# mom-ocean/MOM6

Measured on AMD Instinct MI355X. Metric: simulated-days/wall-sec, higher is better.
Workload: dtype f64

## Files before the change

### include/mom6x.h

```cpp
#ifndef MOM6X_H
#define MOM6X_H

#include <stddef.h>
#include <stdint.h>

#ifdef __cplusplus
extern "C" {
#endif

#define MOM6X_ABI_VERSION 6

typedef struct mom6x_dims {
  int ni, nj, nk;
  int halo;
  int ioff, joff;
  int pitch;
  int slab;
  int i_glob0, j_glob0;
  int ni_glob, nj_glob;
  int reentrant_x, reentrant_y;
} mom6x_dims;

int mom6x_dims_init(mom6x_dims *d, int ni, int nj, int nk, int halo);

// ... 206 lines not shown
int mom6x_prof_reset(mom6x_ctx *ctx);
int mom6x_prof_filter(mom6x_ctx *ctx, const char *prefix);
int mom6x_prof_report(mom6x_ctx *ctx, char *buf, int buflen);

int mom6x_dev_alloc(mom6x_ctx *ctx, double **p, size_t n_doubles);
int mom6x_dev_free(mom6x_ctx *ctx, double *p);
int mom6x_dev_copy(mom6x_ctx *ctx, double *dst, const double *src, size_t n_doubles);
int mom6x_upload(mom6x_ctx *ctx, double *dev, const double *host_f, int stagger, int nk);
int mom6x_download(mom6x_ctx *ctx, double *host_f, const double *dev, int stagger, int nk);


int mom6x_continuity_init(mom6x_ctx *ctx, const mom6x_continuity_params *p);

int mom6x_continuity_stats(mom6x_ctx *ctx, int mode, unsigned long long *out3);

int mom6x_continuity_PPM(mom6x_ctx *ctx,
    const double *u, const double *v, const double *hin, double *h,
    double *uh, double *vh, double dt,
    const double *uhbt, const double *vhbt,
    const double *visc_rem_u, const double *visc_rem_v,
    double *u_cor, double *v_cor, const mom6x_BT_cont *BT_cont,
    double *du_cor, double *dv_cor);


int mom6x_barotropic_init(mom6x_ctx *ctx, const mom6x_barotropic_params *p);

int mom6x_btcalc(mom6x_ctx *ctx, const double *h, const double *h_u, const double *h_v);
int mom6x_btcalc_strict(mom6x_ctx *ctx, const double *h, const double *h_u, const double *h_v);

int mom6x_bt_mass_source(mom6x_ctx *ctx, const double *h, const double *eta, int set_cor);

int mom6x_set_dtbt(mom6x_ctx *ctx, const double *pbce, double gtot_est, double SSH_add,
                   double *dtbt_out);

int mom6x_set_dtbt_pbce_eta(mom6x_ctx *ctx, const double *pbce, const double *eta, double SSH_add, double *dtbt_out);
int mom6x_set_dtbt_pbce(mom6x_ctx *ctx, const double *pbce, double *dtbt_out);

int mom6x_btstep(mom6x_ctx *ctx,
    const double *U_in, const double *V_in, const double *eta_in, double dt,
    const double *bc_accel_u, const double *bc_accel_v,
    const double *taux, const double *tauy, const double *pbce,
    const double *eta_PF_in, const double *U_Cor, const double *V_Cor,
    double *accel_layer_u, double *accel_layer_v, double *eta_out,
    double *uhbtav, double *vhbtav,
    const double *visc_rem_u, const double *visc_rem_v,
    const mom6x_BT_cont *BT_cont,
    const double *taux_bot, const double *tauy_bot,
    const double *uh0, const double *vh0, const double *u_uh0, const double *v_vh0,
    double *etaav);

int mom6x_btstep_warnings(mom6x_ctx *ctx, int reset, long long *count, double *info);

double *mom6x_barotropic_field(mom6x_ctx *ctx, int which);
int mom6x_barotropic_dtbt(mom6x_ctx *ctx, double *get, const double *set);

int mom6x_CoriolisAdv_init(mom6x_ctx *ctx, const mom6x_coriolis_params *p);
int mom6x_CorAdCalc(mom6x_ctx *ctx, const double *u, const double *v, const double *h,
                    const double *uh, const double *vh, double *CAu, double *CAv);

int mom6x_PressureForce_init(mom6x_ctx *ctx, const mom6x_pgf_params *p, const double *Rlay,
                             const double *g_prime);
int mom6x_PressureForce(mom6x_ctx *ctx, const double *h, double *PFu, double *PFv,
                        double *pbce, double *eta);
int mom6x_ALE_PLM_edge_values(mom6x_ctx *ctx, const double *h, const double *Q, int bdry_extrap, double *Q_t, double *Q_b);
int mom6x_ALE_PPM_edge_values(mom6x_ctx *ctx, const double *h, const double *Q, int bdry_extrap, double *Q_t, double *Q_b);
int mom6x_PressureForce_set_tv(mom6x_ctx *ctx, const double *T, const double *S, const mom6x_eos_params *eos);

int mom6x_hor_visc_init(mom6x_ctx *ctx, const mom6x_hor_visc_params *p);
int mom6x_horizontal_viscosity(mom6x_ctx *ctx, const double *u, const double *v, const double *h,
                               double *diffu, double *diffv);

enum mom6x_remap_scheme { MOM6X_REMAP_PCM = 0, MOM6X_REMAP_PLM = 2, MOM6X_REMAP_PPM_H4 = 4, MOM6X_REMAP_PPM_IH4 = 5 };
typedef struct mom6x_remapping_params {
  int    scheme;
  int    boundary_extrapolation;
  int    force_bounds_in_subcell;
  int    force_bounds_in_target;
  int    om4_remap_via_sub_cells;
  int    answer_date;
  double h_neglect;
  double h_neglect_edge;
} mom6x_remapping_params;

int mom6x_ALE_remap_tracers(mom6x_ctx *ctx, const mom6x_remapping_params *p, const double *h_old, const double *h_new,
                            double *const *fields, int nfields);
int mom6x_ALE_remap_set_h_vel(mom6x_ctx *ctx, const double *h_new, double *h_u, double *h_v);
int mom6x_ALE_remap_velocities(mom6x_ctx *ctx, const mom6x_remapping_params *p, const double *h_old_u, const double *h_old_v,
                               const double *h_new_u, const double *h_new_v, double *u, double *v);
int mom6x_ALE_remap_velocities_from_h(mom6x_ctx *ctx, const mom6x_remapping_params *p, const double *h_old, const double *h_new,
                                      double *u, double *v);
int mom6x_ALE_remap_velocities_conserve_ke(mom6x_ctx *ctx, const mom6x_remapping_params *p, const double *h_old_u,
                                           const double *h_old_v, const double *h_new_u, const double *h_new_v,
                                           double *u, double *v);
typedef struct mom6x_regrid_zstar_params {
  double min_thickness;
  double old_grid_weight;
  double depth_of_time_filter_shallow;
  double depth_of_time_filter_deep;
  double Z_ref;
} mom6x_regrid_zstar_params;
int mom6x_ALE_regrid_zstar(mom6x_ctx *ctx, const mom6x_regrid_zstar_params *p, const double *coordinateResolution,
                           const double *h, double *h_new, double *dzRegrid);

enum mom6x_interp_scheme {
  MOM6X_INTERP_P1M_H2 = 0,
  MOM6X_INTERP_PLM = 3, MOM6X_INTERP_PPM_H4 = 5
// ... 247 lines not shown
```

### mom6_amd/abi.py

```python
import ctypes as C
import os

_HERE = os.path.dirname(os.path.abspath(__file__))
LIB_PATH = os.path.join(_HERE, "lib", "libmom6x.so")

c_double_p = C.POINTER(C.c_double)


class Dims(C.Structure):
    _fields_ = [
        ("ni", C.c_int), ("nj", C.c_int), ("nk", C.c_int), ("halo", C.c_int),
        ("ioff", C.c_int), ("joff", C.c_int), ("pitch", C.c_int), ("slab", C.c_int),
        ("i_glob0", C.c_int), ("j_glob0", C.c_int), ("ni_glob", C.c_int), ("nj_glob", C.c_int),
        ("reentrant_x", C.c_int), ("reentrant_y", C.c_int),
    ]

    @property
    def nrows(self):
        return self.nj + 2 * self.halo + 1

    def shape2(self):
        return (self.nrows, self.pitch)

    def shape3(self, nk=None):
# ... 362 lines not shown


class RK2Params(C.Structure):
    _fields_ = [("be", C.c_double), ("begw", C.c_double), ("split_bottom_stress", C.c_int),
                ("BT_use_layer_fluxes", C.c_int), ("store_CAu", C.c_int), ("visc_rem_dt_bug", C.c_int), ("remap_aux", C.c_int),
                ("no_BT_cont", C.c_int)]


def rk2_params_default():
    p = RK2Params()
    p.be, p.begw = 0.6, 0.0
    p.split_bottom_stress = 0
    p.BT_use_layer_fluxes = p.store_CAu = p.visc_rem_dt_bug = 1
    p.remap_aux = 0
    p.no_BT_cont = 0
    return p


VERTVISC_COEF_HOOK = C.CFUNCTYPE(C.c_int, C.c_void_p, C.c_int, C.c_void_p, C.c_void_p, C.c_void_p, C.c_double)
HOR_VISC_HOOK = C.CFUNCTYPE(C.c_int, C.c_void_p, C.c_void_p, C.c_void_p, C.c_void_p, C.c_void_p, C.c_void_p,
                            C.c_void_p, C.c_void_p)


class RK2Hooks(C.Structure):
    _fields_ = [("user", C.c_void_p), ("vertvisc_coef", VERTVISC_COEF_HOOK), ("horizontal_viscosity", HOR_VISC_HOOK)]


RK2_FIELDS = ["CAu", "CAv", "CAu_pred", "CAv_pred", "PFu", "PFv", "diffu", "diffv", "visc_rem_u", "visc_rem_v",
              "u_accel_bt", "v_accel_bt", "u_av", "v_av", "h_av", "pbce", "eta", "eta_PF", "uhbt", "vhbt",
              "taux_bot", "tauy_bot", "BT_h_u", "BT_h_v"]
RK2_HAVE_ETA, RK2_HAVE_DIFFU, RK2_HAVE_U2, RK2_HAVE_CAU, RK2_HAVE_UH, RK2_HAVE_H2 = 1, 2, 4, 8, 16, 32
RK2_FIELDS_2D = {"eta", "eta_PF", "uhbt", "vhbt", "taux_bot", "tauy_bot"}


METRICS = [
    "mask2dT", "mask2dCu", "mask2dCv", "mask2dBu",
    "dxT", "dyT", "IdxT", "IdyT",
    "dxCu", "dyCu", "IdxCu", "IdyCu",
    "dxCv", "dyCv", "IdxCv", "IdyCv",
    "dxBu", "dyBu", "IdxBu", "IdyBu",
    "areaT", "IareaT", "areaBu", "IareaBu",
    "areaCu", "areaCv", "IareaCu", "IareaCv",
    "dy_Cu", "dx_Cv", "bathyT", "CoriolisBu", "Coriolis2Bu",
]
G = {n: i for i, n in enumerate(METRICS)}
G_COUNT = len(METRICS)

MOM6X_OK = 0

_lib = None


ABI_VERSION = 6


def load_library(path=None):
    global _lib
    if _lib is not None and path is None:
        return _lib
    p = path or LIB_PATH
    if not os.path.exists(p):
        raise RuntimeError(
            f"mom6_amd: HIP extension {p} is missing; run `python -c 'import __graft_entry__ as g; g.build()'`. "
            "There is no CPU fallback for the product path.")
    lib = C.CDLL(p, mode=C.RTLD_GLOBAL)
    if lib.mom6x_abi_version() != ABI_VERSION:
        raise RuntimeError(f"mom6_amd: {p} has ABI version {lib.mom6x_abi_version()}, this host mirror was written for "
                           f"{ABI_VERSION} (include/mom6x.h MOM6X_ABI_VERSION); rebuild the library")
    lib.mom6x_last_error.restype = C.c_char_p
    lib.mom6x_ctx_stream.restype = C.c_void_p
    lib.mom6x_ctx_dims.restype = C.POINTER(Dims)
    lib.mom6x_ctx_metrics_dev.restype = C.c_void_p
    for name in ("mom6x_barotropic_field", "mom6x_rk2_field"):
        if hasattr(lib, name):
            getattr(lib, name).restype = C.c_void_p
    if path is None:
        _lib = lib
    return lib


class Mom6xError(RuntimeError):
    pass


def check(lib, rc):
    if rc != MOM6X_OK:
        msg = lib.mom6x_last_error()
        raise Mom6xError(f"mom6x error {rc}: {msg.decode() if msg else ''}")
```

### mom6_amd/csrc/barotropic.hip

```cpp
#include <algorithm>
#include <type_traits>
#include <vector>
#include <cmath>
#include "mom6x_dev.h"

void halo_wrap(mom6x_ctx *c, double *const *fields, const int *staggers, const int *nks, int n);

enum BTW {
  W_q = 0, W_DCor_u, W_DCor_v, W_gtot_E, W_gtot_W, W_gtot_N, W_gtot_S, W_eta, W_eta_PF,
  W_Cor_ref_u, W_Cor_ref_v, W_BT_force_u, W_BT_force_v, W_ubt, W_vbt, W_bt_rem_u, W_bt_rem_v,
  W_uhbt0, W_vhbt0, W_ubt_Cor, W_vbt_Cor, W_uhbt, W_vhbt, W_u_accel_bt, W_v_accel_bt,
  W_eta_src, W_e_anom, W_eta_sum, W_eta_wtd, W_ubt_wtd, W_vbt_wtd, W_eta_pred,
  W_uh0sum, W_vh0sum, W_ubt0, W_vbt0,
  W_f4u, W_f4u_2, W_f4u_3, W_f4u_4, W_f4v, W_f4v_2, W_f4v_3, W_f4v_4,
  W_BTCu,
  W_BTCv = W_BTCu + 10,
  W_BTtmp = W_BTCv + 10,
  W_uhn = W_BTtmp + 12,
  W_vhn,
  W_ubt2, W_vbt2, W_eta_pred2,
  W_COUNT
};

enum BTC { B_FA_EE = 0, B_FA_E0, B_FA_W0, B_FA_WW, B_uBT_WW, B_uBT_EE, B_crvW, B_crvE, B_uh_WW, B_uh_EE };

struct BTState {
  double *frhatu, *frhatv, *IDatu, *IDatv, *ubtav, *vbtav, *eta_cor, *q_D, *D_u_Cor, *D_v_Cor;
  double *work;
  int nstep_last;
  unsigned long long *warn;
  double *warn_info;
  bool la_defer, la_pending;
  const double *la_pbce;
  double la_underflow;
  bool fr_defer, fr_pending;
  const double *fr_hu, *fr_hv;
};

namespace {

__device__ __forceinline__ double *wp(double *work, const Dm &d, int m) { return work + (size_t)m * d.slab; }

__device__ __forceinline__ double find_uhbt(double u, const double *__restrict__ B, size_t c, size_t slab) {
  if (u == 0.0) return 0.0;
  const double uEE = B[B_uBT_EE * slab + c];
  if (u < uEE) return (u - uEE) * B[B_FA_EE * slab + c] + B[B_uh_EE * slab + c];
  if (u < 0.0) return u * (B[B_FA_E0 * slab + c] + B[B_crvE * slab + c] * (u * u));
  const double uWW = B[B_uBT_WW * slab + c];
  if (u <= uWW) return u * (B[B_FA_W0 * slab + c] + B[B_crvW * slab + c] * (u * u));
  return (u - uWW) * B[B_FA_WW * slab + c] + B[B_uh_WW * slab + c];
}

__global__ void k_bt_init_static(Dm d, const double *__restrict__ G, double Z_to_H, double Mean_SL,
                                 double cor_scale, double H_subroundoff, double *q_D, double *D_u_Cor,
                                 double *D_v_Cor, double *IDatu, double *IDatv) {
  const int i = -1 + blockIdx.x * blockDim.x + threadIdx.x;
  const int j = -1 + blockIdx.y * blockDim.y + threadIdx.y;
  if (i > d.ni - 1 || j > d.nj - 1) return;
  const int st = d.pitch;
  const size_t c = ix2(d, i, j);
  const double *bathyT = gm(G, d, MOM6X_G_bathyT), *areaT = gm(G, d, MOM6X_G_areaT), *mT = gm(G, d, MOM6X_G_mask2dT);
  const double *mCu = gm(G, d, MOM6X_G_mask2dCu), *mCv = gm(G, d, MOM6X_G_mask2dCv), *fBu = gm(G, d, MOM6X_G_CoriolisBu);
  if (j >= 0) {
    D_u_Cor[c] = 0.5 * (dmax(Mean_SL + bathyT[c + 1], 0.0) + dmax(Mean_SL + bathyT[c], 0.0)) * Z_to_H;
    if (mCu[c] > 0.) IDatu[c] = mCu[c] * 2.0 / (Z_to_H * ((bathyT[c + 1] + bathyT[c]) + 2.0 * Mean_SL));
    else IDatu[c] = 0.;
  }
  if (i >= 0) {
    D_v_Cor[c] = 0.5 * (dmax(Mean_SL + bathyT[c + st], 0.0) + dmax(Mean_SL + bathyT[c], 0.0)) * Z_to_H;
    if (mCv[c] > 0.) IDatv[c] = mCv[c] * 2.0 / (Z_to_H * ((bathyT[c + st] + bathyT[c]) + 2.0 * Mean_SL));
    else IDatv[c] = 0.;
  }
  if (mT[c] + mT[c + st] + mT[c + 1] + mT[c + 1 + st] > 0.) {
    q_D[c] = 0.25 * (cor_scale * fBu[c]) * ((areaT[c] + areaT[c + 1 + st]) + (areaT[c + 1] + areaT[c + st])) /
// ... 160 lines not shown
  const size_t c = ix2(d, i, j), slab = (size_t)d.slab;
  const double subroundoff = 1e-30;
  const double mC = gm(G, d, DIR ? MOM6X_G_mask2dCv : MOM6X_G_mask2dCu)[c];
  double Ihattot = 0.0;
  if (HF) {
    double hattot = 0.0;
    for (int k = 0; k < nz; k++) hattot = hattot + A.hf[c + (size_t)k * slab];
    Ihattot = mC / (hattot + A.h_neglect);
  }
#define FRH(k) (HF ? A.hf[c + (size_t)(k) * slab] * Ihattot : A.frhat[c + (size_t)(k) * slab])
  double Iwt_tot = 1.0;
  if (!A.wt_uv_bug) {
    double tot = 0.0;
    for (int k = 0; k < nz; k++) {
      double vr = dmin(A.visc_rem[c + k * slab], 1.);
      vr = dmax(vr, 1. - 0.5 * A.Instep / (vr + subroundoff));
      vr = dmax(vr, 0.);
      const double w = FRH(k) * vr;
      tot = (k == 0) ? w : (tot + w);
    }
    Iwt_tot = tot;
    if (fabs(tot) > 0.0) Iwt_tot = mC / tot;
  }
  double ubt_Cor = 0.0, gm_ = 0.0, gp_ = 0.0, uh0sum = 0.0, ubt0 = 0.0, ubt = 0.0, av_rem = 0.0;
  double BT_force = 0.0;
  if (mC > 0.0) {
    BT_force = A.tau[c] * A.RZ_to_H * A.IDat[c] * A.visc_rem[c];
    if (A.tau_bot) BT_force = BT_force - A.tau_bot[c] * A.RZ_to_H * A.IDat[c];
  }
  for (int k = 0; k < nz; k++) {
    const size_t f = c + k * slab;
    const double vrem = A.visc_rem[f], frh = FRH(k);
    double vr = dmin(vrem, 1.);
    vr = dmax(vr, 1. - 0.5 * A.Instep / (vr + subroundoff));
    vr = dmax(vr, 0.);
    double wt = frh * vr;
    if (!A.wt_uv_bug) wt = wt * Iwt_tot;
    ubt_Cor = ubt_Cor + wt * A.U_Cor[f];
    gm_ = gm_ + A.pbce[f] * wt;
    gp_ = gp_ + A.pbce[f + st] * wt;
    if (A.uh0) {
      uh0sum = uh0sum + A.uh0[f];
      ubt0 = ubt0 + (A.visc_rem_u_uh0 ? wt : frh) * A.u_uh0[f];
    }
    ubt = ubt + wt * A.U_in[f];
    BT_force = BT_force + wt * A.bc_accel[f];
    av_rem = av_rem + frh * vrem;
  }
#undef FRH
  A.ubt_Cor[c] = ubt_Cor;
  A.gtot_m[c] = gm_;
  A.gtot_p[c + st] = gp_;
  if (A.uh0) { A.uh0sum[c] = uh0sum; A.ubt0[c] = ubt0; }
  if (fabs(ubt) < A.vel_underflow) ubt = 0.0;
  A.ubt[c] = ubt;
  A.BT_force[c] = BT_force;
  double bt_rem;
  if (A.strong_drag) {
    bt_rem = mC * ((A.nstep * av_rem) / (1.0 + (A.nstep - 1) * av_rem));
  } else {
    bt_rem = 0.0;
    if (mC * av_rem > 0.0) bt_rem = mC * pow(av_rem, A.Instep);
  }
  A.bt_rem[c] = bt_rem;
}

__global__ void k_btcont_copy(Dm d, mom6x_BT_cont BT, double *tmp) {
  const int i = -1 + blockIdx.x * blockDim.x + threadIdx.x;
  const int j = -1 + blockIdx.y * blockDim.y + threadIdx.y;
  if (i > d.ni - 1 || j > d.nj - 1) return;
  const size_t c = ix2(d, i, j), slab = (size_t)d.slab;
  if (j >= 0) {
    tmp[0 * slab + c] = BT.uBT_EE[c]; tmp[1 * slab + c] = BT.uBT_WW[c]; tmp[2 * slab + c] = BT.FA_u_EE[c];
    tmp[3 * slab + c] = BT.FA_u_E0[c]; tmp[4 * slab + c] = BT.FA_u_W0[c]; tmp[5 * slab + c] = BT.FA_u_WW[c];
  }
  if (i >= 0) {
    tmp[6 * slab + c] = BT.vBT_NN[c]; tmp[7 * slab + c] = BT.vBT_SS[c]; tmp[8 * slab + c] = BT.FA_v_NN[c];
    tmp[9 * slab + c] = BT.FA_v_N0[c]; tmp[10 * slab + c] = BT.FA_v_S0[c]; tmp[11 * slab + c] = BT.FA_v_SS[c];
  }
}
__global__ void k_face_areas_as_fits(Dm d, const double *__restrict__ G, double Z_ref, double Z_to_H, double *tmp, const double *__restrict__ eta) {
  const int i = -2 + blockIdx.x * blockDim.x + threadIdx.x;
  const int j = -2 + blockIdx.y * blockDim.y + threadIdx.y;
  if (i > d.ni || j > d.nj) return;
  const int st = d.pitch;
  const size_t c = ix2(d, i, j), slab = (size_t)d.slab;
  const double *bathyT = gm(G, d, MOM6X_G_bathyT);
  const double H1 = eta ? (bathyT[c] * Z_to_H + eta[c]) : ((bathyT[c] + Z_ref) * Z_to_H);
  if (j >= -1) {
    const double H2 = eta ? (bathyT[c + 1] * Z_to_H + eta[c + 1]) : ((bathyT[c + 1] + Z_ref) * Z_to_H);
    double Dat = 0.0;
    if ((H1 > 0.0) && (H2 > 0.0)) Dat = gm(G, d, MOM6X_G_dy_Cu)[c] * (2.0 * H1 * H2) / (H1 + H2);
    tmp[0 * slab + c] = -1.0e100; tmp[1 * slab + c] = 1.0e100;
    tmp[2 * slab + c] = Dat; tmp[3 * slab + c] = Dat; tmp[4 * slab + c] = Dat; tmp[5 * slab + c] = Dat;
  }
  if (i >= -1) {
    const double H2 = eta ? (bathyT[c + st] * Z_to_H + eta[c + st]) : ((bathyT[c + st] + Z_ref) * Z_to_H);
    double Dat = 0.0;
    if ((H1 > 0.0) && (H2 > 0.0)) Dat = gm(G, d, MOM6X_G_dx_Cv)[c] * (2.0 * H1 * H2) / (H1 + H2);
    tmp[6 * slab + c] = -1.0e100; tmp[7 * slab + c] = 1.0e100;
    tmp[8 * slab + c] = Dat; tmp[9 * slab + c] = Dat; tmp[10 * slab + c] = Dat; tmp[11 * slab + c] = Dat;
  }
}
__global__ void k_face_areas_eta(Dm d, const double *__restrict__ G, double Z_to_H, const double *__restrict__ eta, double *Bu, double *Bv,
                                 int isv, int iev, int jsv, int jev) {
  const int i = isv - 2 + blockIdx.x * blockDim.x + threadIdx.x;
// ... 560 lines not shown
  delete s;
  c->bts = nullptr;
}

extern "C" int mom6x_btstep_warnings(mom6x_ctx *c, int reset, long long *count, double *info) {
  REQUIRE(c && c->bts && count, MOM6X_EINVAL, "mom6x_btstep_warnings: barotropic_init has not been called");
  HIPCHK(hipSetDevice(c->device));
  HIPCHK(hipStreamSynchronize(c->stream));
  unsigned long long w[2];
  HIPCHK(hipMemcpy(w, c->bts->warn, sizeof(w), hipMemcpyDeviceToHost));
  *count = (long long)w[0];
  if (info) HIPCHK(hipMemcpy(info, c->bts->warn_info, 4 * sizeof(double), hipMemcpyDeviceToHost));
  if (reset) HIPCHK(hipMemset(c->bts->warn, 0, sizeof(w)));
  return MOM6X_OK;
}

extern "C" int mom6x_barotropic_init(mom6x_ctx *c, const mom6x_barotropic_params *p) {
  REQUIRE(c && p, MOM6X_EINVAL, "mom6x_barotropic_init: null argument");
  REQUIRE(p->bt_thick_scheme >= MOM6X_BT_THICK_FROM_BT_CONT && p->bt_thick_scheme <= MOM6X_BT_THICK_ARITHMETIC, MOM6X_EINVAL,
          "barotropic_init: Unrecognized setting of BT_THICK_SCHEME");
  REQUIRE(c->dims.halo >= 2, MOM6X_EINVAL, "barotropic: halo >= 2 required");
  REQUIRE(p->BTHALO <= c->dims.halo, MOM6X_EINVAL,
          "barotropic_init: BTHALO exceeds the halo of the tile context; create the context with halo = max(NIHALO, BTHALO)");
  REQUIRE(p->min_stencil >= 0 && p->min_stencil <= c->dims.halo, MOM6X_EINVAL, "barotropic_init: bad BT_WIDE_HALO_MIN_STENCIL");
  HIPCHK(hipSetDevice(c->device));
  c->bt = *p;
  const Dm d = c->d;
  if (!c->bts) {
    BTState *s = new BTState();
    memset(s, 0, sizeof(*s));
    const size_t n2 = (size_t)d.slab, n3 = n2 * d.nk;
    double **p3[] = { &s->frhatu, &s->frhatv };
    for (double **q : p3) { HIPCHK(hipMalloc(q, n3 * sizeof(double))); HIPCHK(hipMemsetAsync(*q, 0, n3 * sizeof(double), c->stream)); }
    double **p2[] = { &s->IDatu, &s->IDatv, &s->ubtav, &s->vbtav, &s->eta_cor, &s->q_D, &s->D_u_Cor, &s->D_v_Cor };
    for (double **q : p2) { HIPCHK(hipMalloc(q, n2 * sizeof(double))); HIPCHK(hipMemsetAsync(*q, 0, n2 * sizeof(double), c->stream)); }
    HIPCHK(hipMalloc(&s->work, (size_t)W_COUNT * n2 * sizeof(double)));
    HIPCHK(hipMalloc(&s->warn, 2 * sizeof(unsigned long long))); HIPCHK(hipMemsetAsync(s->warn, 0, 2 * sizeof(unsigned long long), c->stream));
    HIPCHK(hipMalloc(&s->warn_info, 4 * sizeof(double))); HIPCHK(hipMemsetAsync(s->warn_info, 0, 4 * sizeof(double), c->stream));
    c->bts = s;
  }
  BTState *s = c->bts;
  s->nstep_last = 0;
  const dim3 b = blk2();
  KLAUNCH(c, "k_bt_init_static", k_bt_init_static, grid3(d.ni + 1, d.nj + 1, 1, b), b, d, c->G, c->GV.Z_to_H, p->Z_ref,
                     p->BT_Coriolis_scale, c->GV.H_subroundoff, s->q_D, s->D_u_Cor, s->D_v_Cor, s->IDatu, s->IDatv);
  double *f[] = { s->q_D, s->D_u_Cor, s->D_v_Cor };
  const int stg[] = { 3, 1, 2 }, nks[] = { 1, 1, 1 };
  halo_wrap(c, f, stg, nks, 3);
  HIPCHK(hipGetLastError());
  c->bt_init = true;
  return MOM6X_OK;
}

extern "C" double *mom6x_barotropic_field(mom6x_ctx *c, int which) {
  if (!c || !c->bts) return nullptr;
  BTState *s = c->bts;
  if ((which == 3 || which == 4) && bt_frhat_materialize(c)) return nullptr;
  switch (which) {
    case 0: return s->ubtav; case 1: return s->vbtav; case 2: return s->eta_cor; case 3: return s->frhatu;
    case 4: return s->frhatv; case 5: return s->IDatu; case 6: return s->IDatv; case 7: return s->q_D;
    case 8: return s->D_u_Cor; case 9: return s->D_v_Cor; case 10: return s->work;
    default: return nullptr;
  }
}

extern "C" int mom6x_barotropic_dtbt(mom6x_ctx *c, double *get, const double *set) {
  REQUIRE(c && c->bt_init, MOM6X_EINVAL, "mom6x_barotropic_dtbt: Module MOM_barotropic must be initialized before it is used.");
  if (set) { REQUIRE(*set > 0.0, MOM6X_EINVAL, "mom6x_barotropic_dtbt: DTBT must be positive"); c->bt.dtbt = *set; }
  if (get) *get = c->bt.dtbt;
  return MOM6X_OK;
}

extern "C" int mom6x_btcalc_strict(mom6x_ctx *c, const double *h, const double *h_u, const double *h_v) {
  REQUIRE(c && c->bt_init, MOM6X_EINVAL, "btcalc: Module MOM_barotropic must be initialized before it is used.");
  REQUIRE((h_u && h_v) || c->bt.bt_thick_scheme != MOM6X_BT_THICK_FROM_BT_CONT, MOM6X_EINVAL,
          "btcalc: Inconsistent settings of optional arguments and hvel_scheme.");
  return mom6x_btcalc(c, h, h_u, h_v);
}
extern "C" int mom6x_btcalc(mom6x_ctx *c, const double *h, const double *h_u, const double *h_v) {
  REQUIRE(c && c->bt_init, MOM6X_EINVAL, "btcalc: Module MOM_barotropic must be initialized before it is used.");
  REQUIRE((h_u != nullptr) == (h_v != nullptr), MOM6X_EINVAL, "btcalc: Inconsistent settings of optional arguments");
  REQUIRE(h_u || h, MOM6X_EINVAL, "btcalc: h is required when h_u/h_v are absent");
  HIPCHK(hipSetDevice(c->device));
  const Dm d = c->d;
  const dim3 b = blk2();
  c->bts->fr_pending = false;
  if (h_u && c->bts->fr_defer) { c->bts->fr_pending = true; c->bts->fr_hu = h_u; c->bts->fr_hv = h_v; return MOM6X_OK; }
  if (h_u) {
    btcalc_from_faces(c, h_u, h_v);
    HIPCHK(hipGetLastError());
    return MOM6X_OK;
  }
  const int scheme = (c->bt.bt_thick_scheme == MOM6X_BT_THICK_FROM_BT_CONT) ? MOM6X_BT_THICK_HYBRID : c->bt.bt_thick_scheme;
  KLAUNCH(c, "k_btcalc<0>", k_btcalc<0>, grid3(nxa(d.ni + 1, -1), d.nj, 1, b), b, d, c->G, h, h_u, c->bts->frhatu,
                     c->GV.H_subroundoff, c->GV.Z_to_H, scheme);
  KLAUNCH(c, "k_btcalc<1>", k_btcalc<1>, grid3(d.ni, d.nj + 1, 1, b), b, d, c->G, h, h_v, c->bts->frhatv,
                     c->GV.H_subroundoff, c->GV.Z_to_H, scheme);
  HIPCHK(hipGetLastError());
  return MOM6X_OK;
}

extern "C" int mom6x_bt_mass_source(mom6x_ctx *c, const double *h, const double *eta, int set_cor) {
  REQUIRE(c && c->bt_init, MOM6X_EINVAL, "bt_mass_source: Module MOM_barotropic must be initialized before it is used.");
  HIPCHK(hipSetDevice(c->device));
  const Dm d = c->d;
  const dim3 b = blk2();
// ... 42 lines not shown
  HIPCHK(hipStreamSynchronize(c->stream));
  double min_max_dt2 = 1.0e38;
  for (int j = 0; j < d.nj; j++) for (int i = 0; i < d.ni; i++) {
    const double I2 = host[(size_t)(i + d.ioff) + (size_t)(j + d.joff) * d.pitch];
    if (I2 * min_max_dt2 > 1.0) min_max_dt2 = 1.0 / I2;
  }
  const double dgeo_de = 1.0 + fmax(0.0, c->bt.G_extra);
  double dtbt_max = sqrt(min_max_dt2 / dgeo_de);
  { int rc_ = comm_allreduce_scalar(c, &dtbt_max, 0); if (rc_) return rc_; }
  c->bt.dtbt = c->bt.dtbt_fraction * dtbt_max;
  if (dtbt_out) *dtbt_out = c->bt.dtbt;
  return MOM6X_OK;
}

extern "C" int mom6x_btstep(mom6x_ctx *c, const double *U_in, const double *V_in, const double *eta_in, double dt,
                            const double *bc_accel_u, const double *bc_accel_v, const double *taux, const double *tauy,
                            const double *pbce, const double *eta_PF_in, const double *U_Cor, const double *V_Cor,
                            double *accel_layer_u, double *accel_layer_v, double *eta_out, double *uhbtav,
                            double *vhbtav, const double *visc_rem_u, const double *visc_rem_v,
                            const mom6x_BT_cont *BT_cont, const double *taux_bot, const double *tauy_bot,
                            const double *uh0, const double *vh0, const double *u_uh0, const double *v_vh0,
                            double *etaav) {
  REQUIRE(c && c->bt_init, MOM6X_EINVAL, "btstep: Module MOM_barotropic must be initialized before it is used.");
  REQUIRE(U_in && V_in && eta_in && bc_accel_u && bc_accel_v && taux && tauy && pbce && eta_PF_in && U_Cor && V_Cor &&
          accel_layer_u && accel_layer_v && eta_out && uhbtav && vhbtav && visc_rem_u && visc_rem_v,
          MOM6X_EINVAL, "btstep: null mandatory array");
  const bool add_uh0 = (uh0 != nullptr);
  REQUIRE(!add_uh0 || (vh0 && u_uh0 && v_vh0), MOM6X_EINVAL,
          "btstep: vh0, u_uh0, and v_vh0 must be associated if uh0 is used.");
  REQUIRE((taux_bot != nullptr) == (tauy_bot != nullptr), MOM6X_EINVAL, "btstep: taux_bot and tauy_bot come together");
  HIPCHK(hipSetDevice(c->device));
  const Dm d = c->d;
  const mom6x_barotropic_params &P = c->bt;
  BTState *s = c->bts;
  double *work = s->work;
  const size_t slab = (size_t)d.slab;
  const dim3 b = blk2();
  hipStream_t st = c->stream;
  const int is = 0, ie = d.ni - 1, js = 0, je = d.nj - 1;

  const double Idt = 1.0 / dt;
  const bool evolving_face_areas = !BT_cont && P.nonlinear_continuity && P.nonlin_cont_update_period > 0;
  const int stencil = evolving_face_areas ? std::max(2, P.min_stencil) : ((P.min_stencil > 1) ? P.min_stencil : 1);
  const int num_cycles = (P.use_wide_halos && d.halo / stencil >= 1) ? d.halo / stencil : 1;
  const int isvf = is - (num_cycles - 1) * stencil, ievf = ie + (num_cycles - 1) * stencil;
  const int jsvf = js - (num_cycles - 1) * stencil, jevf = je + (num_cycles - 1) * stencil;
  REQUIRE(P.dtbt > 0.0, MOM6X_EINVAL, "btstep: dtbt must be positive (call set_dtbt or set params.dtbt)");
  const int nstep = (int)ceil(dt / P.dtbt - 0.0001);
  s->nstep_last = nstep;
  const double Instep = 1.0 / (double)nstep;
  const double dtbt = dt * Instep;
  const double dgeo_de = 1.0 + P.G_extra;

  HIPCHK(hipMemsetAsync(work, 0, (size_t)W_COUNT * slab * sizeof(double), st));
  KLAUNCH(c, "k_bt_copy_in", k_bt_copy_in, grid3(d.ni + 2 * d.halo + 1, d.nj + 2 * d.halo + 1, 1, b), b, d, work, eta_in,
                     eta_PF_in, s->q_D, s->D_u_Cor, s->D_v_Cor);

  ColArgs Au;
  memset(&Au, 0, sizeof(Au));
  Au.visc_rem = visc_rem_u; Au.frhat = s->frhatu; Au.U_Cor = U_Cor; Au.pbce = pbce; Au.uh0 = uh0; Au.u_uh0 = u_uh0;
  Au.U_in = U_in; Au.bc_accel = bc_accel_u; Au.tau = taux; Au.tau_bot = taux_bot; Au.IDat = s->IDatu;
  Au.ubt_Cor = work + W_ubt_Cor * slab; Au.gtot_m = work + W_gtot_E * slab; Au.gtot_p = work + W_gtot_W * slab;
  Au.uh0sum = work + W_uh0sum * slab; Au.ubt0 = work + W_ubt0 * slab; Au.ubt = work + W_ubt * slab;
  Au.BT_force = work + W_BT_force_u * slab; Au.bt_rem = work + W_bt_rem_u * slab;
  Au.Instep = Instep; Au.RZ_to_H = c->GV.RZ_to_H; Au.vel_underflow = P.vel_underflow; Au.nstep = nstep;
  Au.wt_uv_bug = P.wt_uv_bug; Au.visc_rem_u_uh0 = P.visc_rem_u_uh0; Au.strong_drag = P.strong_drag;
  ColArgs Av = Au;
  Av.visc_rem = visc_rem_v; Av.frhat = s->frhatv; Av.U_Cor = V_Cor; Av.uh0 = vh0; Av.u_uh0 = v_vh0; Av.U_in = V_in;
  Av.bc_accel = bc_accel_v; Av.tau = tauy; Av.tau_bot = tauy_bot; Av.IDat = s->IDatv;
  Av.ubt_Cor = work + W_vbt_Cor * slab; Av.gtot_m = work + W_gtot_N * slab; Av.gtot_p = work + W_gtot_S * slab;
  Av.uh0sum = work + W_vh0sum * slab; Av.ubt0 = work + W_vbt0 * slab; Av.ubt = work + W_vbt * slab;
  Av.BT_force = work + W_BT_force_v * slab; Av.bt_rem = work + W_bt_rem_v * slab;
  if (s->fr_pending) {
    Au.hf = s->fr_hu; Av.hf = s->fr_hv; Au.h_neglect = Av.h_neglect = c->GV.H_subroundoff;
    KLAUNCH(c, "k_bt_col<0>", (k_bt_col<0, true>), grid3(nxa(d.ni + 1, -1), d.nj, 1, b), b, d, c->G, Au);
    KLAUNCH(c, "k_bt_col<1>", (k_bt_col<1, true>), grid3(d.ni, d.nj + 1, 1, b), b, d, c->G, Av);
  } else {
    { const int rcm = bt_frhat_materialize(c); if (rcm) return rcm; }
    KLAUNCH(c, "k_bt_col<0>", (k_bt_col<0, false>), grid3(nxa(d.ni + 1, -1), d.nj, 1, b), b, d, c->G, Au);
    KLAUNCH(c, "k_bt_col<1>", (k_bt_col<1, false>), grid3(d.ni, d.nj + 1, 1, b), b, d, c->G, Av);
  }

  double *tmp = work + W_BTtmp * slab;
  if (BT_cont) KLAUNCH(c, "k_btcont_copy", k_btcont_copy, grid3(d.ni + 1, d.nj + 1, 1, b), b, d, *BT_cont, tmp);
  else KLAUNCH(c, "k_face_areas_as_fits", k_face_areas_as_fits, grid3(d.ni + 3, d.nj + 3, 1, b), b, d, c->G, P.Z_ref, c->GV.Z_to_H, tmp,
               P.nonlinear_continuity ? (const double *)(work + W_eta * slab) : (const double *)nullptr);
  {
    double *f[18]; int stg[18], nks[18];
    for (int m = 0; m < 12; m++) { f[m] = tmp + (size_t)m * slab; stg[m] = (m < 6) ? 1 : 2; nks[m] = 1; }
    double *g[] = { work + W_gtot_E * slab, work + W_gtot_N * slab, work + W_gtot_W * slab, work + W_gtot_S * slab,
                    work + W_ubt_Cor * slab, work + W_vbt_Cor * slab };
    const int gs[] = { 0, 0, 0, 0, 1, 2 };
    for (int m = 0; m < 6; m++) { f[12 + m] = g[m]; stg[12 + m] = gs[m]; nks[12 + m] = 1; }
    halo_wrap(c, f, stg, nks, 18);
  }
  const int hs = 1 + ievf - ie;
  KLAUNCH(c, "k_btcl", k_btcl, grid3(d.ni + 2 * hs + 1, d.nj + 2 * hs + 1, 1, b), b, d, tmp, work + W_BTCu * slab,
                     work + W_BTCv * slab, hs);
  if (add_uh0) KLAUNCH(c, "k_uhbt0", k_uhbt0, grid3(d.ni + 1, d.nj + 1, 1, b), b, d, work, work);

  KLAUNCH(c, "k_find_Cor", k_find_Cor, grid3(ievf - isvf + 3, jevf - jsvf + 3, 1, b), b, d, work, P.Sadourny, isvf, ievf, jsvf, jevf);
  KLAUNCH(c, "k_cor_ref_eta_src", k_cor_ref_eta_src, grid3(d.ni + 1, d.nj + 1, 1, b), b, d, c->G, work, s->eta_cor, Instep,
                     P.bound_BT_corr ? ((BT_cont && P.BT_cont_bounds) ? 1 : 2) : 0, P.maxCFL_BT_cont * Idt, dt, c->GV.Z_to_H, P.Z_ref, P.maxvel);
  {
    std::vector<double *> f = { work + W_eta_PF * slab, work + W_eta_src * slab, work + W_bt_rem_u * slab, work + W_bt_rem_v * slab,
                                work + W_BT_force_u * slab, work + W_BT_force_v * slab };
    std::vector<int> stg = { 0, 0, 1, 2, 1, 2 };
    if (add_uh0) { f.push_back(work + W_uhbt0 * slab); stg.push_back(1); f.push_back(work + W_vhbt0 * slab); stg.push_back(2); }
    f.push_back(work + W_Cor_ref_u * slab); stg.push_back(1); f.push_back(work + W_Cor_ref_v * slab); stg.push_back(2);
    std::vector<int> nks(f.size(), 1);
    halo_wrap(c, f.data(), stg.data(), nks.data(), (int)f.size());
  }

  double dt_filt;
  if (P.dt_bt_filter >= 0.0) dt_filt = 0.5 * fmax(0.0, fmin(P.dt_bt_filter, 2.0 * dt));
  else dt_filt = 0.5 * fmax(0.0, dt * fmin(-P.dt_bt_filter, 2.0));
  const int nfilter = (int)ceil(dt_filt / dtbt);
  const int nt = nstep + nfilter;
  REQUIRE(nt > 0, MOM6X_EINVAL, "btstep: number of barotropic step (nstep+nfilter) is 0");
  std::vector<double> wt_vel(nt + 2, 0.0), wt_eta(nt + 2, 0.0), wt_trans(nt + 2, 0.0), wt_accel(nt + 2, 0.0), wt_accel2(nt + 2, 0.0);
  double sum_wt_vel = 0.0, sum_wt_eta = 0.0, sum_wt_accel = 0.0, sum_wt_trans = 0.0;
  for (int n = 1; n <= nt; n++) {
    if ((n == nstep) || (dt_filt - abs(n - nstep) * dtbt >= 0.0)) { wt_vel[n] = 1.0; wt_eta[n] = 1.0; }
    else if (dtbt + dt_filt - abs(n - nstep) * dtbt > 0.0) { wt_vel[n] = 1.0 + (dt_filt / dtbt) - abs(n - nstep); wt_eta[n] = wt_vel[n]; }
    else { wt_vel[n] = 0.0; wt_eta[n] = 0.0; }
    sum_wt_vel = sum_wt_vel + wt_vel[n]; sum_wt_eta = sum_wt_eta + wt_eta[n];
  }
  for (int n = nt; n >= 1; n--) {
    wt_trans[n] = wt_trans[n + 1] + wt_eta[n];
// ... 120 lines not shown
```

### mom6_amd/dycore.py

```python
import ctypes as C

import numpy as np
import torch

from . import abi
from .abi import BTCont, check, load_library


def _ptr(t):
    if t is None:
        return None
    assert t.is_cuda and t.dtype == torch.float64 and t.is_contiguous(), "need contiguous float64 CUDA tensor"
    return C.c_void_p(t.data_ptr())


class BTContDev:

    def __init__(self, dyc, with_h=True):
        self.f = {n: dyc.zeros2() for n in BTCont._names[:12]}
        self.f["h_u"] = dyc.zeros3() if with_h else None
        self.f["h_v"] = dyc.zeros3() if with_h else None
        self.struct = BTCont()
        for n in BTCont._names:
            t = self.f[n]
# ... 31 lines not shown
                pass
            self.lib.mom6x_ctx_destroy(self.ctx)
            self.ctx = C.c_void_p()

    def __del__(self):
        try:
            self.close()
        except Exception:
            pass

    def zeros2(self):
        with torch.cuda.stream(self.torch_stream()):
            return torch.zeros(self.dims.shape2(), dtype=torch.float64, device=self.device)

    def zeros3(self, nk=None):
        with torch.cuda.stream(self.torch_stream()):
            return torch.zeros(self.dims.shape3(nk), dtype=torch.float64, device=self.device)

    def to_dev(self, a):
        return torch.from_numpy(np.ascontiguousarray(a, dtype=np.float64)).to(self.device)

    def sync(self):
        check(self.lib, self.lib.mom6x_ctx_sync(self.ctx))

    @property
    def stream_ptr(self):
        return self.lib.mom6x_ctx_stream(self.ctx)

    def torch_stream(self):
        return torch.cuda.ExternalStream(self.stream_ptr, device=self.device)

    def continuity_init(self, params=None):
        self.cont_params = params if params is not None else abi.continuity_params_default(self.dims.nk, self.GV.Angstrom_H)
        check(self.lib, self.lib.mom6x_continuity_init(self.ctx, C.byref(self.cont_params)))

    def continuity_PPM(self, u, v, hin, h, uh, vh, dt, uhbt=None, vhbt=None, visc_rem_u=None,
                       visc_rem_v=None, u_cor=None, v_cor=None, BT_cont=None, du_cor=None, dv_cor=None):
        bt = C.byref(BT_cont.struct) if BT_cont is not None else None
        check(self.lib, self.lib.mom6x_continuity_PPM(
            self.ctx, _ptr(u), _ptr(v), _ptr(hin), _ptr(h), _ptr(uh), _ptr(vh), C.c_double(dt),
            _ptr(uhbt), _ptr(vhbt), _ptr(visc_rem_u), _ptr(visc_rem_v), _ptr(u_cor), _ptr(v_cor), bt,
            _ptr(du_cor), _ptr(dv_cor)))

    continuity = continuity_PPM

    def barotropic_init(self, params):
        self.bt_params = params
        check(self.lib, self.lib.mom6x_barotropic_init(self.ctx, C.byref(params)))

    _BT_FIELDS = {"ubtav": (0, 2), "vbtav": (1, 2), "eta_cor": (2, 2), "frhatu": (3, 3), "frhatv": (4, 3),
                  "IDatu": (5, 2), "IDatv": (6, 2), "q_D": (7, 2), "D_u_Cor": (8, 2), "D_v_Cor": (9, 2)}

    def barotropic_field(self, name):
        which, nd = self._BT_FIELDS[name]
        ptr = self.lib.mom6x_barotropic_field(self.ctx, C.c_int(which))
        shape = self.dims.shape2() if nd == 2 else self.dims.shape3()
        return _view(ptr, shape, self.device)

    def btstep_warnings(self, reset=True, warn=True):
        n = C.c_longlong(0)
        info = (C.c_double * 4)()
        check(self.lib, self.lib.mom6x_btstep_warnings(self.ctx, C.c_int(int(reset)), C.byref(n), info))
        first = dict(eta=info[0], minus_bathyT=info[1], i=int(info[2]), j=int(info[3])) if n.value else None
        if n.value and warn:
            import warnings
            warnings.warn("btstep: eta has dropped below bathyT: %24.16E vs. %24.16E at i, j = %d, %d (%d occurrences)" %
                          (info[0], info[1], int(info[2]), int(info[3]), n.value), RuntimeWarning)
        return n.value, first

    def continuity_stats(self, mode=-1):
        out = (C.c_ulonglong * 3)()
        check(self.lib, self.lib.mom6x_continuity_stats(self.ctx, int(mode), out))
        return int(out[0]), int(out[1]), int(out[2])

    def barotropic_dtbt(self, value=None):
        out = C.c_double(0.0)
        check(self.lib, self.lib.mom6x_barotropic_dtbt(self.ctx, C.byref(out), None if value is None else C.byref(C.c_double(value))))
        return out.value

    def btcalc(self, h, h_u=None, h_v=None, may_use_default=True):
        f = self.lib.mom6x_btcalc if may_use_default else self.lib.mom6x_btcalc_strict
        check(self.lib, f(self.ctx, _ptr(h), _ptr(h_u), _ptr(h_v)))

    def set_dtbt_pbce(self, pbce, eta=None, SSH_add=0.0):
        out = C.c_double(0.0)
        check(self.lib, self.lib.mom6x_set_dtbt_pbce_eta(self.ctx, _ptr(pbce), _ptr(eta), C.c_double(SSH_add), C.byref(out)))
        return out.value

    def bt_mass_source(self, h, eta, set_cor):
        check(self.lib, self.lib.mom6x_bt_mass_source(self.ctx, _ptr(h), _ptr(eta), C.c_int(int(set_cor))))

    def set_dtbt(self, pbce=None, gtot_est=0.0, SSH_add=0.0):
        out = C.c_double(0.0)
        check(self.lib, self.lib.mom6x_set_dtbt(self.ctx, _ptr(pbce), C.c_double(gtot_est), C.c_double(SSH_add), C.byref(out)))
        return out.value

    def btstep(self, U_in, V_in, eta_in, dt, bc_accel_u, bc_accel_v, taux, tauy, pbce, eta_PF_in, U_Cor, V_Cor,
               accel_layer_u, accel_layer_v, eta_out, uhbtav, vhbtav, visc_rem_u, visc_rem_v, BT_cont,
               taux_bot=None, tauy_bot=None, uh0=None, vh0=None, u_uh0=None, v_vh0=None, etaav=None):
        check(self.lib, self.lib.mom6x_btstep(
            self.ctx, _ptr(U_in), _ptr(V_in), _ptr(eta_in), C.c_double(dt), _ptr(bc_accel_u), _ptr(bc_accel_v),
            _ptr(taux), _ptr(tauy), _ptr(pbce), _ptr(eta_PF_in), _ptr(U_Cor), _ptr(V_Cor), _ptr(accel_layer_u),
            _ptr(accel_layer_v), _ptr(eta_out), _ptr(uhbtav), _ptr(vhbtav), _ptr(visc_rem_u), _ptr(visc_rem_v),
            C.byref(BT_cont.struct) if BT_cont is not None else None, _ptr(taux_bot), _ptr(tauy_bot), _ptr(uh0), _ptr(vh0), _ptr(u_uh0),
            _ptr(v_vh0), _ptr(etaav)))

    def CoriolisAdv_init(self, params=None):
        self.cor_params = params if params is not None else abi.coriolis_params_default()
        check(self.lib, self.lib.mom6x_CoriolisAdv_init(self.ctx, C.byref(self.cor_params)))

    def CorAdCalc(self, u, v, h, uh, vh, CAu, CAv):
        check(self.lib, self.lib.mom6x_CorAdCalc(self.ctx, _ptr(u), _ptr(v), _ptr(h), _ptr(uh), _ptr(vh), _ptr(CAu), _ptr(CAv)))

    def PressureForce_init(self, params, Rlay, g_prime):
        self.pgf_params = params
        self._Rlay = np.ascontiguousarray(Rlay, dtype=np.float64)
        self._g_prime = np.ascontiguousarray(g_prime, dtype=np.float64)
        check(self.lib, self.lib.mom6x_PressureForce_init(self.ctx, C.byref(params), self._Rlay.ctypes.data_as(C.c_void_p),
                                                          self._g_prime.ctypes.data_as(C.c_void_p)))

    def PressureForce(self, h, PFu, PFv, pbce=None, eta=None):
        check(self.lib, self.lib.mom6x_PressureForce(self.ctx, _ptr(h), _ptr(PFu), _ptr(PFv), _ptr(pbce), _ptr(eta)))

    def ALE_PLM_edge_values(self, h, Q, bdry_extrap, Q_t, Q_b):
        check(self.lib, self.lib.mom6x_ALE_PLM_edge_values(self.ctx, _ptr(h), _ptr(Q), C.c_int(int(bdry_extrap)), _ptr(Q_t), _ptr(Q_b)))

    def set_dyn_pass_width(self, width):
        check(self.lib, self.lib.mom6x_set_dyn_pass_width(self.ctx, C.c_int(int(width))))

    def comm_overlap_btstep(self, on=True):
        check(self.lib, self.lib.mom6x_comm_overlap_btstep(self.ctx, C.c_int(1 if on else 0)))
# ... 342 lines not shown
```

Measured before the change: 0.1947.

## Add column-blocked barotropic column kernel with prefetch and shrink work memset

Adds a templated k_bt_col_cols kernel that walks each column in groups of layers, double-buffering the per-layer loads with scheduling barriers, and specialises it on layer count and on whether uh0 is present. Reorders the barotropic work-plane enum so only the planes that need zeroing sit before W_CLEARED, which lets the per-step memset clear fewer planes. Also exposes work-plane and btcalc-defer entry points. The aim is to cut latency-bound global loads and memset bandwidth; the risk is that some plane moved past W_CLEARED relied on being zeroed.

Result: faster. 0.1972, median of 6 (+1.3%).

```diff
diff --git a/include/mom6x.h b/include/mom6x.h
--- a/include/mom6x.h
+++ b/include/mom6x.h
@@ -282,6 +282,8 @@
 int mom6x_btstep_warnings(mom6x_ctx *ctx, int reset, long long *count, double *info);
 
 double *mom6x_barotropic_field(mom6x_ctx *ctx, int which);
+int mom6x_barotropic_work_planes(mom6x_ctx *ctx);
+int mom6x_btcalc_defer(mom6x_ctx *ctx, int on);
 int mom6x_barotropic_dtbt(mom6x_ctx *ctx, double *get, const double *set);
 
 int mom6x_CoriolisAdv_init(mom6x_ctx *ctx, const mom6x_coriolis_params *p);
diff --git a/mom6_amd/abi.py b/mom6_amd/abi.py
--- a/mom6_amd/abi.py
+++ b/mom6_amd/abi.py
@@ -438,6 +438,7 @@
 
 
 ABI_VERSION = 6
+BT_FIELD_WORK = 10
 
 
 def load_library(path=None):
@@ -460,6 +461,9 @@
     for name in ("mom6x_barotropic_field", "mom6x_rk2_field"):
         if hasattr(lib, name):
             getattr(lib, name).restype = C.c_void_p
+    if hasattr(lib, "mom6x_barotropic_work_planes"):
+        lib.mom6x_barotropic_work_planes.restype = C.c_int
+        lib.mom6x_barotropic_work_planes.argtypes = [C.c_void_p]
     if path is None:
         _lib = lib
     return lib
diff --git a/mom6_amd/csrc/barotropic.hip b/mom6_amd/csrc/barotropic.hip
--- a/mom6_amd/csrc/barotropic.hip
+++ b/mom6_amd/csrc/barotropic.hip
@@ -7,19 +7,24 @@
 void halo_wrap(mom6x_ctx *c, double *const *fields, const int *staggers, const int *nks, int n);
 
 enum BTW {
-  W_q = 0, W_DCor_u, W_DCor_v, W_gtot_E, W_gtot_W, W_gtot_N, W_gtot_S, W_eta, W_eta_PF,
-  W_Cor_ref_u, W_Cor_ref_v, W_BT_force_u, W_BT_force_v, W_ubt, W_vbt, W_bt_rem_u, W_bt_rem_v,
-  W_uhbt0, W_vhbt0, W_ubt_Cor, W_vbt_Cor, W_uhbt, W_vhbt, W_u_accel_bt, W_v_accel_bt,
-  W_eta_src, W_e_anom, W_eta_sum, W_eta_wtd, W_ubt_wtd, W_vbt_wtd, W_eta_pred,
+  W_u_accel_bt = 0, W_v_accel_bt, W_eta_sum, W_eta_wtd, W_ubt_wtd, W_vbt_wtd,
+  W_gtot_E, W_gtot_W, W_gtot_N, W_gtot_S, W_ubt_Cor, W_vbt_Cor, W_BT_force_u, W_BT_force_v, W_bt_rem_u, W_bt_rem_v,
+  W_ubt, W_vbt,
+  W_Cor_ref_u, W_Cor_ref_v, W_eta_src,
+  W_uhbt0, W_vhbt0,
+  W_uhbt, W_vhbt, W_eta_pred,
+  W_uhn,
+  W_vhn,
+  W_ubt2, W_vbt2, W_eta_pred2,
+  W_e_anom,
+  W_BTtmp,
+  W_CLEARED = W_BTtmp + 12,
+  W_q = W_CLEARED, W_DCor_u, W_DCor_v, W_eta, W_eta_PF,
   W_uh0sum, W_vh0sum, W_ubt0, W_vbt0,
   W_f4u, W_f4u_2, W_f4u_3, W_f4u_4, W_f4v, W_f4v_2, W_f4v_3, W_f4v_4,
   W_BTCu,
   W_BTCv = W_BTCu + 10,
-  W_BTtmp = W_BTCv + 10,
-  W_uhn = W_BTtmp + 12,
-  W_vhn,
-  W_ubt2, W_vbt2, W_eta_pred2,
-  W_COUNT
+  W_COUNT = W_BTCv + 10
 };
 
 enum BTC { B_FA_EE = 0, B_FA_E0, B_FA_W0, B_FA_WW, B_uBT_WW, B_uBT_EE, B_crvW, B_crvE, B_uh_WW, B_uh_EE };
@@ -286,6 +291,128 @@
   A.gtot_m[c] = gm_;
   A.gtot_p[c + st] = gp_;
   if (A.uh0) { A.uh0sum[c] = uh0sum; A.ubt0[c] = ubt0; }
+  if (fabs(ubt) < A.vel_underflow) ubt = 0.0;
+  A.ubt[c] = ubt;
+  A.BT_force[c] = BT_force;
+  double bt_rem;
+  if (A.strong_drag) {
+    bt_rem = mC * ((A.nstep * av_rem) / (1.0 + (A.nstep - 1) * av_rem));
+  } else {
+    bt_rem = 0.0;
+    if (mC * av_rem > 0.0) bt_rem = mC * pow(av_rem, A.Instep);
+  }
+  A.bt_rem[c] = bt_rem;
+}
+
+#ifndef BT_COL_G
+#define BT_COL_G 4
+#endif
+template <int DIR, int NKT, bool UH0>
+__global__ void __launch_bounds__(64)
+k_bt_col_cols(Dm d, const double *__restrict__ G, ColArgs A) {
+  constexpr int NK = NK_OF(NKT);
+  const int nk = NK_EXACT(NKT) ? NK : d.nk;
+  const int i = I_BASE((DIR ? 0 : -1)) + blockIdx.x * 64 + threadIdx.x;
+  const int j = (DIR ? -1 : 0) + blockIdx.y;
+  if (i > d.ni - 1 || j > d.nj - 1) return;
+  if (i < ((DIR ? 0 : -1))) return;
+  const int st = DIR ? d.pitch : 1;
+  const size_t c = ix2(d, i, j), slab = (size_t)d.slab;
+  const double subroundoff = 1e-30;
+  constexpr int BG = BT_COL_G;
+  constexpr int NG = (NK + BG - 1) / BG;
+  double hfr[NK];
+#pragma unroll
+  for (int k = 0; k < NK; k++) if (k < nk) hfr[k] = A.hf[c + (size_t)k * slab];
+  double q_vr[2][BG], q_uc[2][BG], q_pm[2][BG], q_pp[2][BG], q_u0[2][BG], q_uu[2][BG], q_ui[2][BG], q_bc[2][BG];
+  auto fetch = [&](int g, int b) {
+#pragma unroll
+    for (int m = 0; m < BG; m++) {
+      const int k = g * BG + m;
+      if (k < NK && k < nk) {
+        const size_t f = c + (size_t)k * slab;
+        q_vr[b][m] = A.visc_rem[f];
+        q_uc[b][m] = A.U_Cor[f];
+        q_pm[b][m] = A.pbce[f];
+        q_pp[b][m] = A.pbce[f + st];
+        if (UH0) { q_u0[b][m] = A.uh0[f]; q_uu[b][m] = A.u_uh0[f]; }
+        q_ui[b][m] = A.U_in[f];
+        q_bc[b][m] = A.bc_accel[f];
+      }
+    }
+  };
+  fetch(0, 0);
+  const double mC = gm(G, d, DIR ? MOM6X_G_mask2dCv : MOM6X_G_mask2dCu)[c];
+  double hattot = 0.0;
+#pragma unroll
+  for (int k = 0; k < NK; k++) if (k < nk) hattot = hattot + hfr[k];
+  const double Ihattot = mC / (hattot + A.h_neglect);
+  double Iwt_tot = 1.0;
+  if (!A.wt_uv_bug) {
+    double tot = 0.0;
+    double p_vr[BG];
+#pragma unroll
+    for (int g = 0; g < NG; g++) {
+#pragma unroll
+      for (int m = 0; m < BG; m++) {
+        const int k = g * BG + m;
+        if (k < NK && k < nk) p_vr[m] = A.visc_rem[c + (size_t)k * slab];
+      }
+      __builtin_amdgcn_sched_barrier(0);
+#pragma unroll
+      for (int m = 0; m < BG; m++) {
+        const int k = g * BG + m;
+        if (k < NK && k < nk) {
+          double vr = dmin(p_vr[m], 1.);
+          vr = dmax(vr, 1. - 0.5 * A.Instep / (vr + subroundoff));
+          vr = dmax(vr, 0.);
+          const double w = (hfr[k] * Ihattot) * vr;
+          tot = (k == 0) ? w : (tot + w);
+        }
+      }
+      __builtin_amdgcn_sched_barrier(0);
+    }
+    Iwt_tot = tot;
+    if (fabs(tot) > 0.0) Iwt_tot = mC / tot;
+  }
+  double ubt_Cor = 0.0, gm_ = 0.0, gp_ = 0.0, uh0sum = 0.0, ubt0 = 0.0, ubt = 0.0, av_rem = 0.0;
+  double BT_force = 0.0;
+  if (mC > 0.0) {
+    BT_force = A.tau[c] * A.RZ_to_H * A.IDat[c] * A.visc_rem[c];
+    if (A.tau_bot) BT_force = BT_force - A.tau_bot[c] * A.RZ_to_H * A.IDat[c];
+  }
+#pragma unroll
+  for (int g = 0; g < NG; g++) {
+    if (g + 1 < NG) fetch(g + 1, (g + 1) & 1);
+    __builtin_amdgcn_sched_barrier(0);
+#pragma unroll
+    for (int m = 0; m < BG; m++) {
+      const int k = g * BG + m;
+      if (k < NK && k < nk) {
+        const double vrem = q_vr[g & 1][m], frh = hfr[k] * Ihattot;
+        double vr = dmin(vrem, 1.);
+        vr = dmax(vr, 1. - 0.5 * A.Instep / (vr + subroundoff));
+        vr = dmax(vr, 0.);
+        double wt = frh * vr;
+        if (!A.wt_uv_bug) wt = wt * Iwt_tot;
+        ubt_Cor = ubt_Cor + wt * q_uc[g & 1][m];
+        gm_ = gm_ + q_pm[g & 1][m] * wt;
+        gp_ = gp_ + q_pp[g & 1][m] * wt;
+        if (UH0) {
+          uh0sum = uh0sum + q_u0[g & 1][m];
+          ubt0 = ubt0 + (A.visc_rem_u_uh0 ? wt : frh) * q_uu[g & 1][m];
+        }
+        ubt = ubt + wt * q_ui[g & 1][m];
+        BT_force = BT_force + wt * q_bc[g & 1][m];
+        av_rem = av_rem + frh * vrem;
+      }
+    }
+    __builtin_amdgcn_sched_barrier(0);
+  }
+  A.ubt_Cor[c] = ubt_Cor;
+  A.gtot_m[c] = gm_;
+  A.gtot_p[c + st] = gp_;
+  if (UH0) { A.uh0sum[c] = uh0sum; A.ubt0[c] = ubt0; }
   if (fabs(ubt) < A.vel_underflow) ubt = 0.0;
   A.ubt[c] = ubt;
   A.BT_force[c] = BT_force;
@@ -952,6 +1079,14 @@
   return MOM6X_OK;
 }
 
+extern "C" int mom6x_btcalc_defer(mom6x_ctx *c, int on) {
+  REQUIRE(c && c->bt_init, MOM6X_EINVAL, "mom6x_btcalc_defer: Module MOM_barotropic must be initialized before it is used.");
+  bt_defer_btcalc(c, on != 0);
+  return MOM6X_OK;
+}
+
+extern "C" int mom6x_barotropic_work_planes(mom6x_ctx *c) { return (c && c->bts) ? (int)W_COUNT : 0; }
+
 extern "C" double *mom6x_barotropic_field(mom6x_ctx *c, int which) {
   if (!c || !c->bts) return nullptr;
   BTState *s = c->bts;
@@ -1100,7 +1235,7 @@
   const double dtbt = dt * Instep;
   const double dgeo_de = 1.0 + P.G_extra;
 
-  HIPCHK(hipMemsetAsync(work, 0, (size_t)W_COUNT * slab * sizeof(double), st));
+  HIPCHK(hipMemsetAsync(work, 0, (size_t)W_CLEARED * slab * sizeof(double), st));
   KLAUNCH(c, "k_bt_copy_in", k_bt_copy_in, grid3(d.ni + 2 * d.halo + 1, d.nj + 2 * d.halo + 1, 1, b), b, d, work, eta_in,
                      eta_PF_in, s->q_D, s->D_u_Cor, s->D_v_Cor);
 
@@ -1121,8 +1256,20 @@
   Av.BT_force = work + W_BT_force_v * slab; Av.bt_rem = work + W_bt_rem_v * slab;
   if (s->fr_pending) {
     Au.hf = s->fr_hu; Av.hf = s->fr_hv; Au.h_neglect = Av.h_neglect = c->GV.H_subroundoff;
-    KLAUNCH(c, "k_bt_col<0>", (k_bt_col<0, true>), grid3(nxa(d.ni + 1, -1), d.nj, 1, b), b, d, c->G, Au);
-    KLAUNCH(c, "k_bt_col<1>", (k_bt_col<1, true>), grid3(d.ni, d.nj + 1, 1, b), b, d, c->G, Av);
+    if (d.nk <= COLS_NK_BOUND) {
+      const dim3 bc(64, 1, 1);
+      const dim3 gu((unsigned)((nxa(d.ni + 1, -1) + 63) / 64), (unsigned)d.nj, 1), gv((unsigned)((d.ni + 63) / 64), (unsigned)(d.nj + 1), 1);
+#define BTCOL(NKT) do {                                                                                                  \
+      if (add_uh0) { KLAUNCH(c, "k_bt_col<0>", (k_bt_col_cols<0, NKT, true>), gu, bc, d, c->G, Au);                        \
+                     KLAUNCH(c, "k_bt_col<1>", (k_bt_col_cols<1, NKT, true>), gv, bc, d, c->G, Av); }                      \
+      else         { KLAUNCH(c, "k_bt_col<0>", (k_bt_col_cols<0, NKT, false>), gu, bc, d, c->G, Au);                       \
+                     KLAUNCH(c, "k_bt_col<1>", (k_bt_col_cols<1, NKT, false>), gv, bc, d, c->G, Av); } } while (0)
+      COLS_NK_DISPATCH(d.nk, BTCOL);
+#undef BTCOL
+    } else {
+      KLAUNCH(c, "k_bt_col<0>", (k_bt_col<0, true>), grid3(nxa(d.ni + 1, -1), d.nj, 1, b), b, d, c->G, Au);
+      KLAUNCH(c, "k_bt_col<1>", (k_bt_col<1, true>), grid3(d.ni, d.nj + 1, 1, b), b, d, c->G, Av);
+    }
   } else {
     { const int rcm = bt_frhat_materialize(c); if (rcm) return rcm; }
     KLAUNCH(c, "k_bt_col<0>", (k_bt_col<0, false>), grid3(nxa(d.ni + 1, -1), d.nj, 1, b), b, d, c->G, Au);
diff --git a/mom6_amd/dycore.py b/mom6_amd/dycore.py
--- a/mom6_amd/dycore.py
+++ b/mom6_amd/dycore.py
@@ -107,6 +107,9 @@
                   "IDatu": (5, 2), "IDatv": (6, 2), "q_D": (7, 2), "D_u_Cor": (8, 2), "D_v_Cor": (9, 2)}
 
     def barotropic_field(self, name):
+        if name == "work":
+            ptr = self.lib.mom6x_barotropic_field(self.ctx, C.c_int(abi.BT_FIELD_WORK))
+            return _view(ptr, (int(self.lib.mom6x_barotropic_work_planes(self.ctx)),) + tuple(self.dims.shape2()), self.device)
         which, nd = self._BT_FIELDS[name]
         ptr = self.lib.mom6x_barotropic_field(self.ctx, C.c_int(which))
         shape = self.dims.shape2() if nd == 2 else self.dims.shape3()
@@ -132,6 +135,9 @@
         out = C.c_double(0.0)
         check(self.lib, self.lib.mom6x_barotropic_dtbt(self.ctx, C.byref(out), None if value is None else C.byref(C.c_double(value))))
         return out.value
+
+    def btcalc_defer(self, on=True):
+        check(self.lib, self.lib.mom6x_btcalc_defer(self.ctx, C.c_int(int(on))))
 
     def btcalc(self, h, h_u=None, h_v=None, may_use_default=True):
         f = self.lib.mom6x_btcalc if may_use_default else self.lib.mom6x_btcalc_strict
```
